# andimarafioti/qwen3-tts-cuda-graphs

Measured on NVIDIA B200. Metric: audio_seconds_per_second, higher is better.
Workload: dtype bf16

## Files before the change

### qwen3_tts_cuda_graphs_b200/csrc/fq3_kernel.cuh

```cuda
#pragma once
#include "fq3_common.cuh"

namespace fq3 {

__device__ __forceinline__ uint32_t smem_u32(const void* p) { return (uint32_t)__cvta_generic_to_shared(p); }

__device__ __forceinline__ void mbar_init(uint64_t* bar, uint32_t count) {
  asm volatile("mbarrier.init.shared::cta.b64 [%0], %1;" ::"r"(smem_u32(bar)), "r"(count) : "memory");
}
__device__ __forceinline__ void mbar_arrive(uint64_t* bar) {
  asm volatile("mbarrier.arrive.shared::cta.b64 _, [%0];" ::"r"(smem_u32(bar)) : "memory");
}
__device__ __forceinline__ void mbar_arrive_expect_tx(uint64_t* bar, uint32_t bytes) {
  asm volatile("mbarrier.arrive.expect_tx.shared::cta.b64 _, [%0], %1;" ::"r"(smem_u32(bar)), "r"(bytes) : "memory");
}
__device__ __forceinline__ bool mbar_try_wait(uint64_t* bar, uint32_t parity) {
  uint32_t ok;
  asm volatile(
      "{\n\t.reg .pred p;\n\t"
      "mbarrier.try_wait.parity.shared::cta.b64 p, [%1], %2;\n\t"
      "selp.u32 %0, 1, 0, p;\n\t}"
      : "=r"(ok)
      : "r"(smem_u32(bar)), "r"(parity)
      : "memory");
// ... 37 lines not shown
  return t;
}
__device__ __forceinline__ int ld_volatile_shared_i32(const int* p) {
  int v;
  asm volatile("ld.volatile.shared.s32 %0, [%1];" : "=r"(v) : "r"(smem_u32(p)) : "memory");
  return v;
}
__device__ __forceinline__ void st_volatile_shared_i32(int* p, int v) {
  asm volatile("st.volatile.shared.s32 [%0], %1;" ::"r"(smem_u32(p)), "r"(v) : "memory");
}
__device__ __forceinline__ uint4 lds128(uint32_t addr) {
  uint4 v;
  asm volatile("ld.shared.v4.u32 {%0, %1, %2, %3}, [%4];" : "=r"(v.x), "=r"(v.y), "=r"(v.z), "=r"(v.w) : "r"(addr));
  return v;
}

__device__ __forceinline__ LLWord ll_ld(const LLWord* p) {
  LLWord w;
  asm volatile("ld.relaxed.gpu.global.v2.u32 {%0, %1}, [%2];" : "=r"(w.x), "=r"(w.y) : "l"(p) : "memory");
  return w;
}
__device__ __forceinline__ void ll_ld2(const LLWord* p, LLWord& a, LLWord& b) {
  asm volatile("ld.relaxed.gpu.global.v4.u32 {%0, %1, %2, %3}, [%4];" : "=r"(a.x), "=r"(a.y), "=r"(b.x), "=r"(b.y) : "l"(p) : "memory");
}
__device__ __forceinline__ void ll_st(LLWord* p, uint32_t payload, uint32_t ep) {
  const unsigned long long val = ((unsigned long long)ep << 32) | payload;
  asm volatile("red.relaxed.gpu.global.max.u64 [%0], %1;" ::"l"(p), "l"(val) : "memory");
}
__device__ __forceinline__ void ll_st2(LLWord* p, uint32_t pay0, uint32_t pay1, uint32_t ep) {
  ll_st(p, pay0, ep);
  ll_st(p + 1, pay1, ep);
}
__device__ __forceinline__ void ll_stf(LLWord* p, float v, uint32_t ep) { ll_st(p, __float_as_uint(v), ep); }

__device__ __forceinline__ float bf16r(float x) { return __bfloat162float(__float2bfloat16_rn(x)); }
__device__ __forceinline__ float bf_lo(uint32_t w) { return __uint_as_float(w << 16); }
__device__ __forceinline__ float bf_hi(uint32_t w) { return __uint_as_float(w & 0xffff0000u); }
__device__ __forceinline__ uint32_t pack_bf16x2(float lo, float hi) {
  __nv_bfloat162 v = __floats2bfloat162_rn(lo, hi);
  return *reinterpret_cast<uint32_t*>(&v);
}
__device__ __forceinline__ float warp_sum(float v) {
#pragma unroll
  for (int o = 16; o > 0; o >>= 1) v += __shfl_xor_sync(0xffffffffu, v, o);
  return v;
}
__device__ __forceinline__ float warp_max(float v) {
#pragma unroll
  for (int o = 16; o > 0; o >>= 1) v = fmaxf(v, __shfl_xor_sync(0xffffffffu, v, o));
  return v;
}
struct Smem {
  uint64_t* full;
  uint64_t* empty;
  int* ctl;
  float* red;
  unsigned char* scratch;
  KindDesc* kinds;
  UnitDesc* units;
  Phase* prog;
  unsigned char* gam;
  unsigned char* xbuf;
  unsigned char* ring;
};

__device__ __forceinline__ Smem carve_smem(unsigned char* base, const LaunchParams& p) {
// ... 407 lines not shown
  cbar_sync();
  if (tprof) prof_acc(p, 2, *tprof);
}

template <int UNITS, int JC>
__device__ __noinline__ void load_x_rows(const LaunchParams& p, uint32_t flags, const LLWord* in, int ld, uint32_t gam, float eps,
                                         int K, int M, uint32_t ep_in, int pidx, uint32_t xs, uint32_t red) {
  load_x_rows_impl<UNITS, JC, false>(p, flags, in, ld, gam, eps, K, M, ep_in, pidx, xs, red, nullptr);
}

__device__ __forceinline__ float2 tree_parts(float y0, float y1, uint32_t pa, uint32_t stride, int wpg) {
  float P0[8], P1[8];
#pragma unroll
  for (int g = 0; g < 8; ++g) {
    float s0 = 0.f, s1 = 0.f;
    if (g != 0 && g < wpg) { const float2 v = lds_f32x2(pa + (uint32_t)g * stride); s0 = v.x; s1 = v.y; }
    if (g + 8 < wpg) { const float2 v = lds_f32x2(pa + (uint32_t)(g + 8) * stride); s0 += v.x; s1 += v.y; }
    if (g == 0) { s0 += y0; s1 += y1; }
    P0[g] = s0; P1[g] = s1;
  }
  return make_float2(((P0[0] + P0[1]) + (P0[2] + P0[3])) + ((P0[4] + P0[5]) + (P0[6] + P0[7])),
                     ((P1[0] + P1[1]) + (P1[2] + P1[3])) + ((P1[4] + P1[5]) + (P1[6] + P1[7])));
}

template <bool PROF>
__device__ __forceinline__ void gemv_phase_consume(const Ctx& c, const Phase& ph, const LaunchParams& p, RingCur& cur, RingCur& gcur, uint32_t& gst,
                                                   int pidx, uint32_t ep) {
  const int tid = threadIdx.x, warp = tid >> 5, lane = tid & 31;
  RingCur cur0 = cur, gcur0 = gcur;
  const uint32_t kda = c.kinds + (uint32_t)ph.kind * (uint32_t)sizeof(KindDesc);
  const uint4 k0 = lds128(kda);
  const uint4 k3 = lds128(kda + 48u);
  const uint4 ud = lds128(c.units + (uint32_t)(ph.kind * kConsumerWarps + warp) * (uint32_t)sizeof(UnitDesc));
  if (k3.x == 0u) return;
  const uint32_t flags = k0.w;
  const int Kq = (int)k0.z;
  const LLWord* in = reinterpret_cast<const LLWord*>(((unsigned long long)k0.y << 32) | k0.x);
  const uint32_t ep_in = (pidx == 0 && ep == p.epoch_base + 1) ? 0u : ep - 1;
  const bool norm = (flags & F_PRENORM) != 0;
  if (PROF) prof_mark(p, pidx, 0);
  if (PROF) prof_cta_time(p, pidx, 0);
  if (PROF) prof_warp_time(p, pidx, 0);

  const uint4 k6 = lds128(kda + 96u);
  const bool fast = k6.w != 0u;
  const bool poller = tid < kPollThreads;
  const bool have0 = poller && tid < Kq, have1 = poller && tid + kPollThreads < Kq, have2 = poller && tid + 2 * kPollThreads < Kq;
  const LLWord* src = in + 2 * tid;
  uint4 w0 = make_uint4(0u, ep_in, 0u, ep_in), w1 = w0, w2 = w0;
  if (fast) {
    if (have0) w0 = ll_ld_pair(src);
    if (have1) w1 = ll_ld_pair(src + 2 * kPollThreads);
    if (have2) w2 = ll_ld_pair(src + 4 * kPollThreads);
  }

  const uint4 k1 = lds128(kda + 16u);
  const uint4 k2 = lds128(kda + 32u);
  const uint4 k4 = lds128(kda + 64u);
  const uint4 k5 = lds128(kda + 80u);
  const int M = (int)k6.x, n_words = (int)k6.y, K = (int)k6.z;
  FQ3_ASSERT(M >= 1 && M <= kMaxRows && (K & 63) == 0 && (M == 1 ? 2 * K * 2 : M * (int)xrow_stride(K)) <= p.xbuf_bytes, pidx, 300000 + M);
  struct { int g, grp0, n_stages; } sb = {(int)k3.x, (int)k3.y, (int)k4.w};
  const int wpg = (int)k3.z, gpr = (int)k3.w, spg = (int)k4.x, ro_shift = (int)k4.z;
  const int g8 = lane >> 2, t = lane & 3;
  const int wgrp = (int)ud.x, kp = (int)ud.y;
  const bool w_act = wgrp < gpr;
  int ch0 = (int)ud.z, ch1 = (int)ud.w;
  uint32_t gsrc = c.gam + (uint32_t)gcur0.slot * (uint32_t)c.gam_bytes + (uint32_t)tid * 8u;
  uint32_t gfullb = c.gfull + (uint32_t)gcur0.slot * 8u, gemptyb = c.gempty + (uint32_t)gcur0.slot * 8u;
  const uint32_t glap = gcur0.lap;
  if (norm) gcur0.advance(1, kGammaSlots);
  float eps = __uint_as_float(k5.x);
  float inv_k = __uint_as_float(k5.y);
  const uint32_t par = gst & 1u;
  const uint32_t xs = c.xs + (fast ? par * c.xhalf : 0u);
  uint32_t xdst0 = xs + xquad_off(tid), xdst1 = xs + xquad_off(tid + kPollThreads), xdst2 = xs + xquad_off(tid + 2 * kPollThreads);
  uint32_t xrow = xs + (uint32_t)min(g8, M - 1) * xrow_stride(K) + (uint32_t)t * 16u;
  const uint32_t lane_w = (uint32_t)lane * 16u;
  const uint32_t pbase = c.scratch + par * (uint32_t)(kConsumerWarps * 32 * 8);
  uint32_t pdst = pbase + (uint32_t)((wgrp * wpg + kp) * 32 + lane) * 8u;
  LLWord* out = reinterpret_cast<LLWord*>(((unsigned long long)k1.y << 32) | k1.x);
  const LLWord* resp = reinterpret_cast<const LLWord*>(((unsigned long long)k1.w << 32) | k1.z);
  const uint32_t* biasp = reinterpret_cast<const uint32_t*>(((unsigned long long)k2.y << 32) | k2.x);
  const int ldout = (int)k2.z, ldres = (int)k2.w;
  const bool f_lane = w_act && kp == 0 && g8 < M && (ro_shift == 1 || (t & 1) == 0);
  const int f_sub = (ro_shift == 1) ? t : (t >> 1);
  const int wpgrp = (int)k5.w;
  int gi = wgrp;
  int f_word = (sb.grp0 + gi) * wpgrp + f_sub;
  uint32_t res0 = 0u, bias0 = 0u;
  const bool g_ok0 = w_act && gi < sb.g;
  if (f_lane && g_ok0 && f_word < n_words) {
    if (flags & F_RESID) res0 = ll_ld(resp + (size_t)g8 * ldres + f_word).x;
    if (flags & F_BIAS) bias0 = __ldg(biasp + f_word);
// ... 77 lines not shown
          const float4 r0 = lds_f32x4(c.red), r1 = lds_f32x4(c.red + 16u);
          static_assert(kPollWarps == 8, "the RMSNorm reduction reads eight per-warp sums");
          tot = ((r0.x + r0.y) + (r0.z + r0.w)) + ((r1.x + r1.y) + (r1.z + r1.w));
        }
        const float rs = rsqrtf(fmaf(tot, inv_k, eps));
        const bool wr = (flags & F_WRITE_NORMED) && blockIdx.x == 0;
        if (have0) {
          const uint32_t y0 = norm_pair(w0.x, rs, g0.x), y1 = norm_pair(w0.z, rs, g0.y);
          xquad_store(xdst0, y0, y1);
          if (wr) reinterpret_cast<uint2*>(p.bufs[BUF_HID])[tid] = make_uint2(y0, y1);
        }
        if (have1) {
          const uint32_t y0 = norm_pair(w1.x, rs, g1.x), y1 = norm_pair(w1.z, rs, g1.y);
          xquad_store(xdst1, y0, y1);
          if (wr) reinterpret_cast<uint2*>(p.bufs[BUF_HID])[tid + kPollThreads] = make_uint2(y0, y1);
        }
        if (have2) {
          const uint32_t y0 = norm_pair(w2.x, rs, g2.x), y1 = norm_pair(w2.z, rs, g2.y);
          xquad_store(xdst2, y0, y1);
          if (wr) reinterpret_cast<uint2*>(p.bufs[BUF_HID])[tid + 2 * kPollThreads] = make_uint2(y0, y1);
        }
        __syncwarp();
        if (lane == 0) mbar_arrive_a(gemptyb);
      }
    }
    if (PROF) prof_warp_time(p, pidx, 6);
    cbar_sync();
    if (PROF) prof_warp_time(p, pidx, 1);
  } else {
    if (norm && !mbar_try_wait_a(gfullb, glap)) {
      Spin spin;
      while (!mbar_try_wait_a(gfullb, glap)) spin.tick(p, DE_FULL_WAIT, pidx, 100);
    }
    load_x_rows<1, 3>(p, flags, in, (int)lds_u32(kda + 112u), gsrc - (uint32_t)tid * 8u, eps, K, M, ep_in, pidx, c.xs, c.red);
    if (norm) {
      if (lane == 0) mbar_arrive_a(gemptyb);
    }
  }
  if (PROF) prof_mark(p, pidx, 1);

#pragma unroll 1
  for (int r = 0; r < n_rounds; ++r) {
    if (r != 0) cbar_sync();
    gi = r * gpr + wgrp;
    if (!(w_act && gi < sb.g)) continue;
    if (r != 0) {
      my = cur0;
      my.advance(gi * spg + (ch0 >> 5), c.n_stages);
      const uint32_t fb = c.full + (uint32_t)my.slot * 8u;
      Spin spin;
      while (!mbar_try_wait_a(fb, my.lap)) spin.tick(p, DE_FULL_WAIT, pidx, my.slot);
      wa0 = c.ring + lane_w + (uint32_t)my.slot * kStageBytes + (uint32_t)(ch0 & (kStageChunks - 1)) * kBlockBytes;
    }
    float acc[4] = {0.f, 0.f, 0.f, 0.f}, acc2[4] = {0.f, 0.f, 0.f, 0.f};
    int ch = ch0;
    uint32_t wa = wa0, xa = xa0;
    if (PROF && r == 0) prof_mark(p, pidx, 8);
    if (PROF && r == 0) prof_warp_time(p, pidx, 2);
    if (r == 0 && npre > 0) {
      uint4 xv = lds128(xa);
#pragma unroll
      for (int i = 0; i < kPre; ++i) {
        if (i < npre) {
          uint4 xn = xv;
          if (ch0 + i + 1 < ch1) xn = lds128(xa + (uint32_t)(i + 1) * kXBlock);
          mma_bf16(acc, xv.x, xv.x, xv.y, xv.y, wreg[i].x, wreg[i].y);
          mma_bf16(acc2, xv.z, xv.z, xv.w, xv.w, wreg[i].z, wreg[i].w);
// ... 81 lines not shown
#pragma unroll
            for (int o = 4; o <= 16; o <<= 1) {
              s0 += __shfl_xor_sync(0xffffffffu, s0, o);
              s1 += __shfl_xor_sync(0xffffffffu, s1, o);
            }
            if (g8 == m) { r0 = s0; r1 = s1; }
          }
          y0 = r0; y1 = r1;
        }
      }
    }
    if (PROF && r == 0) prof_mark(p, pidx, 10, kProfLeader);
    if (kp == 0) {
      if (r != 0) {
        f_word = (sb.grp0 + gi) * wpgrp + f_sub;
        if (f_lane && f_word < n_words) {
          if (flags & F_RESID) res0 = ll_ld(resp + (size_t)g8 * ldres + f_word).x;
          if (flags & F_BIAS) bias0 = __ldg(biasp + f_word);
        }
      }
      float lo, hi;
      if (flags & F_SWIGLU) {
        const float e = bf16r(bf16r(silu_f(bf16r(y0))) * bf16r(y1));
        lo = e;
        hi = __shfl_down_sync(0xffffffffu, e, 1);
      } else {
        lo = y0; hi = y1;
        if (flags & F_BIAS) { lo += bf_lo(bias0); hi += bf_hi(bias0); }
        lo = bf16r(lo); hi = bf16r(hi);
        if (flags & F_SILU) { lo = bf16r(silu_f(lo)); hi = bf16r(silu_f(hi)); }
      }
      if (flags & F_RESID) { lo = bf16r(bf_lo(res0) + lo); hi = bf16r(bf_hi(res0) + hi); }
      if (PROF) prof_cta_time(p, pidx, 1);
      if (f_lane && f_word < n_words) ll_st(out + (size_t)g8 * ldout + f_word, pack_bf16x2(lo, hi), ep);
      if (PROF && r == 0) prof_mark(p, pidx, 11, kProfLeader);
      if (PROF && r == 0) prof_warp_time(p, pidx, 7);
      if (wpg == 1) {
        __syncwarp();
        if (lane == 0) {
          int rs = cur0.slot + gi * spg;
          while (rs >= c.n_stages) rs -= c.n_stages;
          for (int s2 = 0; s2 < spg; ++s2) {
            mbar_arrive_a(c.empty + (uint32_t)rs * 8u);
            if (++rs == c.n_stages) rs = 0;
          }
        }
      }
    }
  }
  cur0.advance(sb.n_stages, c.n_stages);
  cur = cur0;
  gcur = gcur0;
  gst = ((gst & 1u) ^ 1u) | (fast ? 0u : 2u);
  if (PROF) prof_mark(p, pidx, 3, kProfLeader);
  if (PROF) prof_warp_time(p, pidx, 4);
}


struct KindRegs {
  const LLWord* in; int Kq, flags; LLWord* out; const LLWord* res; const uint32_t* bias; int ldout, ldres;
  int g, grp0, wpg, gpr, spg, nch, ro_shift, n_stages; float eps, inv_k; int n_rounds, wpgrp, M, n_words, K, fast, ldin, norm;
};
__device__ __forceinline__ KindRegs load_kind(uint32_t kda) {
  const uint4 k0 = lds128(kda), k1 = lds128(kda + 16u), k2 = lds128(kda + 32u), k3 = lds128(kda + 48u), k4 = lds128(kda + 64u),
              k5 = lds128(kda + 80u), k6 = lds128(kda + 96u), k7 = lds128(kda + 112u);
  KindRegs r;
  r.in = reinterpret_cast<const LLWord*>(((unsigned long long)k0.y << 32) | k0.x); r.Kq = (int)k0.z; r.flags = (int)k0.w;
// ... 274 lines not shown
__device__ __forceinline__ int num_splits(int L, int cap) {
  const int want = (L + kSplitLen - 1) / kSplitLen;
  return max(1, min(want, cap));
}

struct RopeRegs {
  uint2 g2, c2, s2;
};
__device__ __forceinline__ RopeRegs rope_load(const bf16* gamma, const bf16* cosp, const bf16* sinp, int lane) {
  RopeRegs r;
  const uint64_t keep = policy_evict_last();
  r.g2 = ldg_keep_u2(gamma + lane * 4, keep);
  r.c2 = ldg_keep_u2(cosp + lane * 4, keep);
  r.s2 = ldg_keep_u2(sinp + lane * 4, keep);
  return r;
}
__device__ __forceinline__ void head_norm_rope(float (&x)[4], const RopeRegs& rr, float eps, int lane) {
  const uint2 g2 = rr.g2, c2 = rr.c2, s2 = rr.s2;
  float ss = x[0] * x[0] + x[1] * x[1] + x[2] * x[2] + x[3] * x[3];
  ss = warp_sum(ss);
  const float rs = rsqrtf(ss * (1.f / kHeadDim) + eps);
  const float g[4] = {bf_lo(g2.x), bf_hi(g2.x), bf_lo(g2.y), bf_hi(g2.y)};
  const float c[4] = {bf_lo(c2.x), bf_hi(c2.x), bf_lo(c2.y), bf_hi(c2.y)};
  const float sn[4] = {bf_lo(s2.x), bf_hi(s2.x), bf_lo(s2.y), bf_hi(s2.y)};
  float y[4];
#pragma unroll
  for (int i = 0; i < 4; ++i) y[i] = bf16r(bf16r(x[i] * rs) * g[i]);
#pragma unroll
  for (int i = 0; i < 4; ++i) {
    const float partner = __shfl_xor_sync(0xffffffffu, y[i], 16);
    const float rot = (lane < 16) ? -partner : partner;
    x[i] = bf16r(bf16r(y[i] * c[i]) + bf16r(rot * sn[i]));
  }
}

__device__ __forceinline__ void ll_head_wait(const LLWord* src, uint32_t ep, LLWord& a, LLWord& b, const LaunchParams& p, int phase) {
  ll_ld2(src, a, b);
  if (ep == 0) return;
  Spin spin;
  unsigned tries = 0;
  while (__any_sync(0xffffffffu, a.y != ep || b.y != ep)) {
    if (++tries > 4) __nanosleep(40);
    spin.tick(p, DE_LL_WAIT, phase, (int)ep);
    ll_ld2(src, a, b);
  }
}

constexpr int kGq = 2;
constexpr int kAttnPre = 2;
constexpr int kAttnShort = 2 * kAttnPre * kConsumerWarps;

template <bool PROF>
__device__ __forceinline__ void attn_row(const Phase& ph, const LaunchParams& p, unsigned char* smem_base, const Group& gr, int r, int kvh, int sp,
                                      int nsplit, uint32_t ep, int pidx) {
  const Smem sm = carve_smem(smem_base, p);
  const StackRt& S = p.stacks[ph.stack];
  const int warp = threadIdx.x >> 5, lane = threadIdx.x & 31;
  const int gq = S.nq / S.nkv;
  const int qb = ph.stack == ST_TALKER ? BUF_TQKV : BUF_PQKV, ab = ph.stack == ST_TALKER ? BUF_TATT : BUF_PATT;
  const LLWord* qkv = reinterpret_cast<const LLWord*>(p.bufs[qb]) + (size_t)gr.first_row * p.ld[qb];
  const int ldq = p.ld[qb];
  constexpr int HW = kHeadDim / 2;
  const size_t head_base = (((size_t)ph.layer * S.n_slots + gr.slot) * S.nkv + kvh) * (size_t)S.max_pos * kHeadDim;
  bf16* Kc = S.kcache + head_base;
  bf16* Vc = S.vcache + head_base;
  const int pos = gr.pos0 + r;
// ... 2 lines not shown
  FQ3_ASSERT(r >= 0 && r < kMaxRows && sp >= 0 && sp < nsplit && nsplit <= kMaxSplits, pidx, 210000 + sp);
  const int per = (L + nsplit - 1) / nsplit;
  const int a = gr.n_pad + sp * per;
  const int b = min(a + per, pos + 1);
  float* qs = reinterpret_cast<float*>(sm.scratch);
  uint4* fresh = reinterpret_cast<uint4*>(sm.scratch + 1024);
  float* wp = reinterpret_cast<float*>(sm.scratch + 1024 + 4096);
  const uint32_t ep_in = ep - 1;
  const int hw = lane >> 4, dl = lane & 15;
  if (PROF) prof_mark(p, pidx, 0);

  uint4 kpre[kAttnPre], vpre[kAttnPre];
#pragma unroll
  for (int u = 0; u < kAttnPre; ++u) {
    const int i = a + warp * 2 + hw + u * 2 * kConsumerWarps;
    kpre[u] = make_uint4(0u, 0u, 0u, 0u);
    vpre[u] = kpre[u];
    if (i < b && i < gr.pos0) {
      kpre[u] = __ldcg(reinterpret_cast<const uint4*>(Kc + (size_t)i * kHeadDim) + dl);
      vpre[u] = __ldcg(reinterpret_cast<const uint4*>(Vc + (size_t)i * kHeadDim) + dl);
    }
  }
  cbar_sync();
  if (threadIdx.x < kGq * kAttnShort) wp[threadIdx.x] = -INFINITY;

  for (int it = warp; it < gq + 2 * (r + 1); it += kConsumerWarps) {
    if (it < gq) {
      const int rp = min(max(pos + gr.rope_delta, 0), S.rope_len - 1);
      const LLWord* src = qkv + (size_t)r * ldq + (kvh * gq + it) * HW + lane * 2;
      const RopeRegs rr = rope_load(reinterpret_cast<const bf16*>(p.arena + (size_t)ph.g_off * 16), S.rope_cos + (size_t)rp * kHeadDim,
                                    S.rope_sin + (size_t)rp * kHeadDim, lane);
      LLWord w0, w1;
      ll_head_wait(src, ep_in, w0, w1, p, pidx);
      float x[4] = {bf_lo(w0.x), bf_hi(w0.x), bf_lo(w1.x), bf_hi(w1.x)};
      head_norm_rope(x, rr, S.eps, lane);
      const float scale = rsqrtf((float)kHeadDim);
      *reinterpret_cast<float4*>(qs + it * kHeadDim + lane * 4) = make_float4(x[0] * scale, x[1] * scale, x[2] * scale, x[3] * scale);
    } else {
      const int r2 = (it - gq) >> 1;
      const bool is_v = ((it - gq) & 1) != 0;
      const int kp = gr.pos0 + r2;
      if (kp >= a && kp < b) {
        const LLWord* row = qkv + (size_t)r2 * ldq;
        uint2* f = reinterpret_cast<uint2*>(fresh + (size_t)r2 * 32);
        if (is_v) {
          const LLWord* vsrc = row + (S.nq + S.nkv + kvh) * HW + lane * 2;
          LLWord v0, v1;
          ll_head_wait(vsrc, ep_in, v0, v1, p, pidx);
          const uint2 vv = make_uint2(v0.x, v1.x);
          *reinterpret_cast<uint2*>(Vc + (size_t)kp * kHeadDim + lane * 4) = vv;
          f[32 + lane] = vv;
        } else {
          const int rp = min(max(kp + gr.rope_delta, 0), S.rope_len - 1);
          const LLWord* ksrc = row + (S.nq + kvh) * HW + lane * 2;
          const RopeRegs rr = rope_load(reinterpret_cast<const bf16*>(p.arena + (size_t)ph.b_off * 16), S.rope_cos + (size_t)rp * kHeadDim,
                                        S.rope_sin + (size_t)rp * kHeadDim, lane);
          LLWord k0, k1;
          ll_head_wait(ksrc, ep_in, k0, k1, p, pidx);
          float x[4] = {bf_lo(k0.x), bf_hi(k0.x), bf_lo(k1.x), bf_hi(k1.x)};
          head_norm_rope(x, rr, S.eps, lane);
          const uint2 kk = make_uint2(pack_bf16x2(x[0], x[1]), pack_bf16x2(x[2], x[3]));
          *reinterpret_cast<uint2*>(Kc + (size_t)kp * kHeadDim + lane * 4) = kk;
          f[lane] = kk;
        }
      }
    }
  }
  cbar_sync();
  if (PROF) prof_mark(p, pidx, 1);

  float qr[kGq][8];
#pragma unroll
  for (int j = 0; j < kGq; ++j) {
    const float4 q0 = *reinterpret_cast<const float4*>(qs + j * kHeadDim + dl * 8);
    const float4 q1 = *reinterpret_cast<const float4*>(qs + j * kHeadDim + dl * 8 + 4);
    qr[j][0] = q0.x; qr[j][1] = q0.y; qr[j][2] = q0.z; qr[j][3] = q0.w;
    qr[j][4] = q1.x; qr[j][5] = q1.y; qr[j][6] = q1.z; qr[j][7] = q1.w;
  }
  if (b - a <= kAttnShort) {
    float* sc = wp;
    uint4* vst = reinterpret_cast<uint4*>(wp + kGq * kAttnShort);
    float sv[2][kGq];
    uint4 vv[2];
    int idx[2];
#pragma unroll
    for (int u = 0; u < 2; ++u) {
      const int i = a + warp * 2 + hw + u * 2 * kConsumerWarps;
      idx[u] = (i < b) ? i - a : -1;
      uint4 kk = make_uint4(0u, 0u, 0u, 0u);
      vv[u] = kk;
      if (i < b) {
        if (i >= gr.pos0) {
          const uint4* f = fresh + (size_t)(i - gr.pos0) * 32;
          kk = f[dl];
          vv[u] = f[16 + dl];
        } else {
          kk = kpre[u];
          vv[u] = vpre[u];
        }
      }
      const float k[8] = {bf_lo(kk.x), bf_hi(kk.x), bf_lo(kk.y), bf_hi(kk.y), bf_lo(kk.z), bf_hi(kk.z), bf_lo(kk.w), bf_hi(kk.w)};
#pragma unroll
      for (int j = 0; j < kGq; ++j) {
        float t = 0.f;
#pragma unroll
        for (int d = 0; d < 8; ++d) t = fmaf(qr[j][d], k[d], t);
        sv[u][j] = t;
      }
    }
#pragma unroll
    for (int o = 8; o > 0; o >>= 1) {
#pragma unroll
      for (int u = 0; u < 2; ++u) {
#pragma unroll
        for (int j = 0; j < kGq; ++j) sv[u][j] += __shfl_xor_sync(0xffffffffu, sv[u][j], o);
      }
    }
#pragma unroll
    for (int u = 0; u < 2; ++u) {
      vst[(warp * 2 + hw + u * 2 * kConsumerWarps) * 16 + dl] = vv[u];
      if (idx[u] >= 0 && dl < kGq) sc[dl * kAttnShort + idx[u]] = (dl == 0) ? sv[u][0] : sv[u][1];
    }
    if (PROF) prof_mark(p, pidx, 2);
    cbar_sync();
    float* pr = reinterpret_cast<float*>(vst + kAttnShort * 16);
    const int n = b - a;
    const int n4 = (n + 3) >> 2;
    if (threadIdx.x < kGq * kAttnShort) {
      const int j = threadIdx.x / kAttnShort, i = threadIdx.x - j * kAttnShort;
      const float4* s4 = reinterpret_cast<const float4*>(sc + j * kAttnShort);
      float Mx = -INFINITY;
      for (int g4 = 0; g4 < n4; ++g4) {
        const float4 v = s4[g4];
        Mx = fmaxf(Mx, fmaxf(fmaxf(v.x, v.y), fmaxf(v.z, v.w)));
      }
      pr[threadIdx.x] = expf(sc[threadIdx.x] - Mx);
      if (i == 0) pr[kGq * kAttnShort + j] = Mx;
    }
    cbar_sync();
    if (threadIdx.x < gq * HW) {
      const int j = threadIdx.x / HW, wd = threadIdx.x - j * HW;
      const int qh = kvh * gq + j;
      const int row = gr.first_row + r;
      const float4* p4 = reinterpret_cast<const float4*>(pr + j * kAttnShort);
      const float Mx = pr[kGq * kAttnShort + j];
      const uint32_t* vw = reinterpret_cast<const uint32_t*>(vst) + wd;
      float Lsum = 0.f, O0 = 0.f, O1 = 0.f;
#pragma unroll 3
      for (int g4 = 0; g4 < n4; ++g4) {
        const float4 v = p4[g4];
        const uint32_t w0 = vw[(4 * g4) * HW], w1 = vw[(4 * g4 + 1) * HW], w2 = vw[(4 * g4 + 2) * HW], w3 = vw[(4 * g4 + 3) * HW];
        Lsum += v.x; O0 = fmaf(v.x, bf_lo(w0), O0); O1 = fmaf(v.x, bf_hi(w0), O1);
        Lsum += v.y; O0 = fmaf(v.y, bf_lo(w1), O0); O1 = fmaf(v.y, bf_hi(w1), O1);
        Lsum += v.z; O0 = fmaf(v.z, bf_lo(w2), O0); O1 = fmaf(v.z, bf_hi(w2), O1);
        Lsum += v.w; O0 = fmaf(v.w, bf_lo(w3), O0); O1 = fmaf(v.w, bf_hi(w3), O1);
      }
      if (nsplit == 1) {
        const float y0 = bf16r(Lsum > 0.f ? O0 / Lsum : 0.f), y1 = bf16r(Lsum > 0.f ? O1 / Lsum : 0.f);
        ll_st(reinterpret_cast<LLWord*>(p.bufs[ab]) + (size_t)row * p.ld[ab] + qh * HW + wd, pack_bf16x2(y0, y1), ep);
      } else {
        LLWord* dst = p.attn_part + (((size_t)row * S.nq + qh) * kMaxSplits + sp) * kPartStride;
        if (wd == 0) ll_st2(dst, __float_as_uint(Mx), __float_as_uint(Lsum), ep);
        ll_st2(dst + 4 + 2 * wd, __float_as_uint(O0), __float_as_uint(O1), ep);
      }
    }
    if (PROF) prof_mark(p, pidx, 3);
    return;
  }
  float m_run[kGq], l_run[kGq], acc[kGq][8];
#pragma unroll
  for (int j = 0; j < kGq; ++j) {
    m_run[j] = -INFINITY; l_run[j] = 0.f;
#pragma unroll
    for (int d = 0; d < 8; ++d) acc[j][d] = 0.f;
  }
  auto step = [&](const uint4& kk, const uint4& vv, bool valid) {
    const float k[8] = {bf_lo(kk.x), bf_hi(kk.x), bf_lo(kk.y), bf_hi(kk.y), bf_lo(kk.z), bf_hi(kk.z), bf_lo(kk.w), bf_hi(kk.w)};
    const float v[8] = {bf_lo(vv.x), bf_hi(vv.x), bf_lo(vv.y), bf_hi(vv.y), bf_lo(vv.z), bf_hi(vv.z), bf_lo(vv.w), bf_hi(vv.w)};
    float s[kGq];
#pragma unroll
    for (int j = 0; j < kGq; ++j) {
      float t = 0.f;
#pragma unroll
      for (int d = 0; d < 8; ++d) t = fmaf(qr[j][d], k[d], t);
      s[j] = t;
    }
#pragma unroll
    for (int o = 8; o > 0; o >>= 1) {
#pragma unroll
      for (int j = 0; j < kGq; ++j) s[j] += __shfl_xor_sync(0xffffffffu, s[j], o);
    }
    if (valid) {
#pragma unroll
      for (int j = 0; j < kGq; ++j) {
        const float m_new = fmaxf(m_run[j], s[j]);
        const float corr = expf(m_run[j] - m_new);
        const float pj = expf(s[j] - m_new);
        l_run[j] = l_run[j] * corr + pj;
#pragma unroll
        for (int d = 0; d < 8; ++d) acc[j][d] = fmaf(pj, v[d], acc[j][d] * corr);
        m_run[j] = m_new;
      }
    }
  };
  {
    int u = 0;
#pragma unroll 1
    for (int i0 = a + warp * 2; i0 < b; i0 += 2 * kConsumerWarps, ++u) {
      const int i = i0 + hw;
      const bool valid = i < b;
      uint4 kk = make_uint4(0u, 0u, 0u, 0u), vv = kk;
      if (valid) {
        if (i >= gr.pos0) {
          const uint4* f = fresh + (size_t)(i - gr.pos0) * 32;
          kk = f[dl];
          vv = f[16 + dl];
        } else if (u < kAttnPre) {
          kk = (u == 0) ? kpre[0] : kpre[1];
          vv = (u == 0) ? vpre[0] : vpre[1];
        } else {
          kk = __ldcg(reinterpret_cast<const uint4*>(Kc + (size_t)i * kHeadDim) + dl);
          vv = __ldcg(reinterpret_cast<const uint4*>(Vc + (size_t)i * kHeadDim) + dl);
        }
      }
// ... 9 lines not shown
    const float c_o = (m_o == -INFINITY) ? 0.f : expf(m_o - m_new);
    float o8[8];
#pragma unroll
    for (int d = 0; d < 8; ++d) {
      const float a_o = __shfl_xor_sync(0xffffffffu, acc[j][d], 16);
      o8[d] = acc[j][d] * c_s + a_o * c_o;
    }
    const float l_new = l_run[j] * c_s + l_o * c_o;
    if (hw == 0) {
      float* w = wp + ((size_t)warp * kGq + j) * kPartStride;
      if (dl == 0) { w[0] = m_new; w[1] = l_new; }
      *reinterpret_cast<float4*>(w + 4 + dl * 8) = make_float4(o8[0], o8[1], o8[2], o8[3]);
      *reinterpret_cast<float4*>(w + 8 + dl * 8) = make_float4(o8[4], o8[5], o8[6], o8[7]);
    }
  }
  if (PROF) prof_mark(p, pidx, 2);
  cbar_sync();
  if (threadIdx.x < gq * HW) {
    const int j = threadIdx.x / HW, wd = threadIdx.x - j * HW;
    const int qh = kvh * gq + j;
    const int row = gr.first_row + r;
    const int nw = min(kConsumerWarps, (b - a + 1) >> 1);
    float Mx = -INFINITY;
    for (int w = 0; w < nw; ++w) Mx = fmaxf(Mx, wp[((size_t)w * kGq + j) * kPartStride]);
    float Lsum = 0.f, O0 = 0.f, O1 = 0.f;
    for (int w = 0; w < nw; ++w) {
      const float* q = wp + ((size_t)w * kGq + j) * kPartStride;
      const float f = (q[0] == -INFINITY) ? 0.f : expf(q[0] - Mx);
      Lsum += q[1] * f;
      const float2 o2 = *reinterpret_cast<const float2*>(q + 4 + 2 * wd);
      O0 += o2.x * f; O1 += o2.y * f;
    }
    if (nsplit == 1) {
      const float y0 = bf16r(Lsum > 0.f ? O0 / Lsum : 0.f), y1 = bf16r(Lsum > 0.f ? O1 / Lsum : 0.f);
      ll_st(reinterpret_cast<LLWord*>(p.bufs[ab]) + (size_t)row * p.ld[ab] + qh * HW + wd, pack_bf16x2(y0, y1), ep);
    } else {
      LLWord* dst = p.attn_part + (((size_t)row * S.nq + qh) * kMaxSplits + sp) * kPartStride;
      if (wd == 0) ll_st2(dst, __float_as_uint(Mx), __float_as_uint(Lsum), ep);
      ll_st2(dst + 4 + 2 * wd, __float_as_uint(O0), __float_as_uint(O1), ep);
    }
  }
  if (PROF) prof_mark(p, pidx, 3);
}

__device__ __forceinline__ void combine_step(float& Mx, float& Lsum, float& O0, float& O1, float ms, float ls, float a0, float a1) {
  if (ms != -INFINITY) {
    const float m_new = fmaxf(Mx, ms);
    const float c_old = (Mx == -INFINITY) ? 0.f : expf(Mx - m_new);
    const float c_new = expf(ms - m_new);
    Lsum = Lsum * c_old + ls * c_new;
    O0 = O0 * c_old + a0 * c_new;
    O1 = O1 * c_old + a1 * c_new;
    Mx = m_new;
  }
}

__device__ __forceinline__ void attn_combine(const Phase& ph, const LaunchParams& p, const Group& gr, int r, int kvh, int nsplit, uint32_t ep,
                                          int pidx) {
  const StackRt& S = p.stacks[ph.stack];
  const int gq = S.nq / S.nkv;
  const int ab = ph.stack == ST_TALKER ? BUF_TATT : BUF_PATT;
  constexpr int HW = kHeadDim / 2;
  if (threadIdx.x < gq * HW) {
    const int j = threadIdx.x / HW, wd = threadIdx.x - j * HW;
    const int qh = kvh * gq + j;
    const int row = gr.first_row + r;
    const LLWord* src = p.attn_part + (((size_t)row * S.nq + qh) * kMaxSplits) * kPartStride;
    float Mx = -INFINITY, Lsum = 0.f, O0 = 0.f, O1 = 0.f;
// ... 267 lines not shown
  }
#pragma unroll 1
  for (int pass = 0; pass < 2; ++pass) {
#pragma unroll 1
    for (int item = first; item < total; item += step) {
      int base = 0;
      bool found = false;
      for (int g = 0; g < ng && !found; ++g) {
        const Group gr = get_group(ph, p, g, frame_pos);
        for (int r = 0; r < gr.nrows; ++r) {
          int nsplit; bool multi;
          const int nitems = row_items(gr, r, nsplit, multi);
          if (item < base + nitems) {
            const int it = item - base;
            if (multi) {
              if constexpr (WIDE) {
                if (pass == 0) attn_item_multi(ph, p, smem_base, gr, it, nsplit, ep, pidx);
              }
            } else {
              const int kvh = small_div(it, nsplit), sp = it - kvh * nsplit;
              if (pass == 0) attn_row<PROF>(ph, p, smem_base, gr, r, kvh, sp, nsplit, ep, pidx);
              else if (nsplit > 1 && sp == 0) attn_combine(ph, p, gr, r, kvh, nsplit, ep, pidx);
            }
            found = true;
            break;
          }
          base += nitems;
        }
      }
    }
  }
}

__device__ __forceinline__ uint32_t f2key(float f) {
  uint32_t u = __float_as_uint(f);
  return (u & 0x80000000u) ? ~u : (u | 0x80000000u);
}
__device__ __forceinline__ float key2f(uint32_t k) {
  uint32_t u = (k & 0x80000000u) ? (k & 0x7fffffffu) : ~k;
  return __uint_as_float(u);
}
__device__ __forceinline__ uint4 philox4x32_10(uint4 c, uint2 k) {
#pragma unroll
  for (int i = 0; i < 10; ++i) {
    const uint32_t hi0 = __umulhi(0xD2511F53u, c.x), lo0 = 0xD2511F53u * c.x;
    const uint32_t hi1 = __umulhi(0xCD9E8D57u, c.z), lo1 = 0xCD9E8D57u * c.z;
    c = make_uint4(hi1 ^ c.y ^ k.x, lo1, hi0 ^ c.w ^ k.y, lo0);
    k.x += 0x9E3779B9u;
    k.y += 0xBB67AE85u;
  }
  return c;
}

struct SampleScratch {
  float* sl;
  unsigned* hist;
  float* redf;
  int* redi;
};
__device__ __forceinline__ SampleScratch sample_scratch(unsigned char* scratch) {
  SampleScratch s;
  s.sl = reinterpret_cast<float*>(scratch);
  s.hist = reinterpret_cast<unsigned*>(scratch + 20 * 1024);
  s.redf = reinterpret_cast<float*>(scratch + 21 * 1024);
  s.redi = reinterpret_cast<int*>(scratch + 21 * 1024 + 256);
  return s;
// ... 729 lines not shown
          int* sconst = reinterpret_cast<int*>(smem_raw + kStreamConstOffset);
          sconst[tid] = __ldcg(&st->n_pad);
          sconst[kMaxWide + tid] = __ldcg(&st->rope_delta);
        } else {
          done = (int)ll_wait(&st->ctl[0], ep0, p, -2);
          pos = (int)ll_wait(&st->ctl[1], ep0, p, -2);
        }
        frame_pos[tid] = pos;
        frame_done[tid] = done;
      }
      cbar_sync();
      if (p.mode == MODE_FRAMES && iter > 0) {
        int all_done = 1;
        for (int b = 0; b < p.n_rows; ++b) all_done &= (frame_done[b] != 0);
        if (all_done) {
          if (tid == 0) st_volatile_shared_i32(&sm.ctl[0], -1);
          break;
        }
      }
    }
    for (int i = 0; i < p.n_phases; ++i) {
      const Phase ph = load_phase(sm.prog, i);
      const uint32_t ep = ep0 + (uint32_t)i + 1u;
      switch (ph.type) {
        case PH_GEMV:
          if constexpr (WIDE) gemv_phase_consume_wide(c, ph, p, cur, gcur, gst, i, ep);
          else gemv_phase_consume<PROF>(c, ph, p, cur, gcur, gst, i, ep);
          break;
        case PH_ATTN:
          if constexpr (WIDE) {
            long long tp = (FQ3_WIDE_PROF && p.prof) ? clock64() : 0ll;
            attn_phase<PROF, true>(ph, p, smem_raw, ep, i, frame_pos);
            prof_acc(p, 4, tp);
          } else {
            attn_phase<PROF, false>(ph, p, smem_raw, ep, i, frame_pos);
          }
          break;
        case PH_SAMPLE:
          if constexpr (WIDE) {
            long long tp = (FQ3_WIDE_PROF && p.prof) ? clock64() : 0ll;
            sample_phase<WIDE>(ph, p, smem_raw, ep, i, frame_done);
            prof_acc(p, 5, tp);
          } else {
            sample_phase<WIDE>(ph, p, smem_raw, ep, i, frame_done);
          }
          break;
        default: if (tid == 0) device_fault(p, DE_BAD_PHASE, i, ph.type); break;
      }
    }
  }
}

__global__ void fq3_tile_weights_kernel(const bf16* __restrict__ W, uint4* __restrict__ out, int N, int K) {
  const long pieces = (long)((N + 7) / 8) * K;
  for (long idx = blockIdx.x * (long)blockDim.x + threadIdx.x; idx < pieces; idx += (long)gridDim.x * blockDim.x) {
    const long grp = idx / K;
    const int pc = (int)(idx - grp * K);
    const int ch = pc >> 5, ln = pc & 31, r8 = ln >> 2, t = ln & 3;
    const long row = grp * 8 + r8;
    uint4 v = make_uint4(0u, 0u, 0u, 0u);
    if (row < N) {
      const uint32_t* src = reinterpret_cast<const uint32_t*>(W + (size_t)row * K + ch * kChunkK) + t;
      v = make_uint4(__ldg(src), __ldg(src + 4), __ldg(src + 8), __ldg(src + 12));
    }
    out[idx] = v;
  }
// ... 182 lines not shown
```

Before: 46.31.

## Fold predictor attention into the following GEMV by staging outputs in shared memory

Adds a pred_attn_fold path for the predictor stack in single-row decode mode. Every CTA redundantly computes the short-context attention for all KV heads and writes the result directly into the shared-memory x buffer of the next GEMV phase. Flag bits in gst make that GEMV skip its global polling and x loading, and add an acq_rel fence before stores so the KV-cache writes are ordered. This removes a global LL write/poll round trip and a phase boundary, at the cost of redundant attention compute in every CTA. It also factors existing attention helpers into shared inline functions.

```diff
diff --git a/qwen3_tts_cuda_graphs_b200/csrc/fq3_kernel.cuh b/qwen3_tts_cuda_graphs_b200/csrc/fq3_kernel.cuh
--- a/qwen3_tts_cuda_graphs_b200/csrc/fq3_kernel.cuh
+++ b/qwen3_tts_cuda_graphs_b200/csrc/fq3_kernel.cuh
@@ -93,6 +93,9 @@
   ll_st(p + 1, pay1, ep);
 }
 __device__ __forceinline__ void ll_stf(LLWord* p, float v, uint32_t ep) { ll_st(p, __float_as_uint(v), ep); }
+
+__device__ __forceinline__ void fence_acq_rel_gpu() { asm volatile("fence.acq_rel.gpu;" ::: "memory"); }
+__device__ __forceinline__ void prefetch_l1(const void* ptr) { asm volatile("prefetch.global.L1 [%0];" ::"l"(ptr)); }
 
 __device__ __forceinline__ float bf16r(float x) { return __bfloat162float(__float2bfloat16_rn(x)); }
 __device__ __forceinline__ float bf_lo(uint32_t w) { return __uint_as_float(w << 16); }
@@ -566,7 +569,10 @@
   const uint4 k0 = lds128(kda);
   const uint4 k3 = lds128(kda + 48u);
   const uint4 ud = lds128(c.units + (uint32_t)(ph.kind * kConsumerWarps + warp) * (uint32_t)sizeof(UnitDesc));
-  if (k3.x == 0u) return;
+  if (k3.x == 0u) {
+    gst &= 3u;
+    return;
+  }
   const uint32_t flags = k0.w;
   const int Kq = (int)k0.z;
   const LLWord* in = reinterpret_cast<const LLWord*>(((unsigned long long)k0.y << 32) | k0.x);
@@ -578,7 +584,8 @@
 
   const uint4 k6 = lds128(kda + 96u);
   const bool fast = k6.w != 0u;
-  const bool poller = tid < kPollThreads;
+  const bool staged = (gst & 4u) != 0u;
+  const bool poller = !staged && tid < kPollThreads;
   const bool have0 = poller && tid < Kq, have1 = poller && tid + kPollThreads < Kq, have2 = poller && tid + 2 * kPollThreads < Kq;
   const LLWord* src = in + 2 * tid;
   uint4 w0 = make_uint4(0u, ep_in, 0u, ep_in), w1 = w0, w2 = w0;
@@ -593,7 +600,7 @@
   const uint4 k4 = lds128(kda + 64u);
   const uint4 k5 = lds128(kda + 80u);
   const int M = (int)k6.x, n_words = (int)k6.y, K = (int)k6.z;
-  FQ3_ASSERT(M >= 1 && M <= kMaxRows && (K & 63) == 0 && (M == 1 ? 2 * K * 2 : M * (int)xrow_stride(K)) <= p.xbuf_bytes, pidx, 300000 + M);
+  FQ3_ASSERT(M >= 1 && M <= kMaxRows && (K & 63) == 0 && (M == 1 ? 2 * K * 2 : M * (int)xrow_stride(K)) <= p.xbuf_bytes && !(staged && norm), pidx, 300000 + M);
   struct { int g, grp0, n_stages; } sb = {(int)k3.x, (int)k3.y, (int)k4.w};
   const int wpg = (int)k3.z, gpr = (int)k3.w, spg = (int)k4.x, ro_shift = (int)k4.z;
   const int g8 = lane >> 2, t = lane & 3;
@@ -737,7 +744,7 @@
       Spin spin;
       while (!mbar_try_wait_a(gfullb, glap)) spin.tick(p, DE_FULL_WAIT, pidx, 100);
     }
-    load_x_rows<1, 3>(p, flags, in, (int)lds_u32(kda + 112u), gsrc - (uint32_t)tid * 8u, eps, K, M, ep_in, pidx, c.xs, c.red);
+    if (!staged) load_x_rows<1, 3>(p, flags, in, (int)lds_u32(kda + 112u), gsrc - (uint32_t)tid * 8u, eps, K, M, ep_in, pidx, c.xs, c.red);
     if (norm) {
       if (lane == 0) mbar_arrive_a(gemptyb);
     }
@@ -885,7 +892,10 @@
       }
       if (flags & F_RESID) { lo = bf16r(bf_lo(res0) + lo); hi = bf16r(bf_hi(res0) + hi); }
       if (PROF) prof_cta_time(p, pidx, 1);
-      if (f_lane && f_word < n_words) ll_st(out + (size_t)g8 * ldout + f_word, pack_bf16x2(lo, hi), ep);
+      if (f_lane && f_word < n_words) {
+        if (gst & 8u) fence_acq_rel_gpu();
+        ll_st(out + (size_t)g8 * ldout + f_word, pack_bf16x2(lo, hi), ep);
+      }
       if (PROF && r == 0) prof_mark(p, pidx, 11, kProfLeader);
       if (PROF && r == 0) prof_warp_time(p, pidx, 7);
       if (wpg == 1) {
@@ -1226,6 +1236,52 @@
     const float rot = (lane < 16) ? -partner : partner;
     x[i] = bf16r(bf16r(y[i] * c[i]) + bf16r(rot * sn[i]));
   }
+}
+
+__device__ __forceinline__ float4 q_head(LLWord w0, LLWord w1, const RopeRegs& rr, float eps, int lane) {
+  float x[4] = {bf_lo(w0.x), bf_hi(w0.x), bf_lo(w1.x), bf_hi(w1.x)};
+  head_norm_rope(x, rr, eps, lane);
+  const float scale = rsqrtf((float)kHeadDim);
+  return make_float4(x[0] * scale, x[1] * scale, x[2] * scale, x[3] * scale);
+}
+__device__ __forceinline__ uint2 k_head(LLWord k0, LLWord k1, const RopeRegs& rr, float eps, int lane) {
+  float x[4] = {bf_lo(k0.x), bf_hi(k0.x), bf_lo(k1.x), bf_hi(k1.x)};
+  head_norm_rope(x, rr, eps, lane);
+  return make_uint2(pack_bf16x2(x[0], x[1]), pack_bf16x2(x[2], x[3]));
+}
+__device__ __forceinline__ float qk_partial(const float (&q)[8], uint4 kk) {
+  const float k[8] = {bf_lo(kk.x), bf_hi(kk.x), bf_lo(kk.y), bf_hi(kk.y), bf_lo(kk.z), bf_hi(kk.z), bf_lo(kk.w), bf_hi(kk.w)};
+  float t = 0.f;
+#pragma unroll
+  for (int d = 0; d < 8; ++d) t = fmaf(q[d], k[d], t);
+  return t;
+}
+template <int N>
+__device__ __forceinline__ void half_sums(float (&v)[N]) {
+#pragma unroll
+  for (int o = 8; o > 0; o >>= 1) {
+#pragma unroll
+    for (int n = 0; n < N; ++n) v[n] += __shfl_xor_sync(0xffffffffu, v[n], o);
+  }
+}
+__device__ __forceinline__ float scores_max(const float* sc, int n4) {
+  const float4* s4 = reinterpret_cast<const float4*>(sc);
+  float Mx = -INFINITY;
+  for (int g4 = 0; g4 < n4; ++g4) {
+    const float4 v = s4[g4];
+    Mx = fmaxf(Mx, fmaxf(fmaxf(v.x, v.y), fmaxf(v.z, v.w)));
+  }
+  return Mx;
+}
+__device__ __forceinline__ void pv_step4(float4 v, uint32_t w0, uint32_t w1, uint32_t w2, uint32_t w3, float& Lsum, float& O0, float& O1) {
+  Lsum += v.x; O0 = fmaf(v.x, bf_lo(w0), O0); O1 = fmaf(v.x, bf_hi(w0), O1);
+  Lsum += v.y; O0 = fmaf(v.y, bf_lo(w1), O0); O1 = fmaf(v.y, bf_hi(w1), O1);
+  Lsum += v.z; O0 = fmaf(v.z, bf_lo(w2), O0); O1 = fmaf(v.z, bf_hi(w2), O1);
+  Lsum += v.w; O0 = fmaf(v.w, bf_lo(w3), O0); O1 = fmaf(v.w, bf_hi(w3), O1);
+}
+__device__ __forceinline__ uint32_t attn_word(float Lsum, float O0, float O1) {
+  const float y0 = bf16r(Lsum > 0.f ? O0 / Lsum : 0.f), y1 = bf16r(Lsum > 0.f ? O1 / Lsum : 0.f);
+  return pack_bf16x2(y0, y1);
 }
 
 __device__ __forceinline__ void ll_head_wait(const LLWord* src, uint32_t ep, LLWord& a, LLWord& b, const LaunchParams& p, int phase) {
@@ -1294,10 +1350,7 @@
                                     S.rope_sin + (size_t)rp * kHeadDim, lane);
       LLWord w0, w1;
       ll_head_wait(src, ep_in, w0, w1, p, pidx);
-      float x[4] = {bf_lo(w0.x), bf_hi(w0.x), bf_lo(w1.x), bf_hi(w1.x)};
-      head_norm_rope(x, rr, S.eps, lane);
-      const float scale = rsqrtf((float)kHeadDim);
-      *reinterpret_cast<float4*>(qs + it * kHeadDim + lane * 4) = make_float4(x[0] * scale, x[1] * scale, x[2] * scale, x[3] * scale);
+      *reinterpret_cast<float4*>(qs + it * kHeadDim + lane * 4) = q_head(w0, w1, rr, S.eps, lane);
     } else {
       const int r2 = (it - gq) >> 1;
       const bool is_v = ((it - gq) & 1) != 0;
@@ -1319,9 +1372,7 @@
                                         S.rope_sin + (size_t)rp * kHeadDim, lane);
           LLWord k0, k1;
           ll_head_wait(ksrc, ep_in, k0, k1, p, pidx);
-          float x[4] = {bf_lo(k0.x), bf_hi(k0.x), bf_lo(k1.x), bf_hi(k1.x)};
-          head_norm_rope(x, rr, S.eps, lane);
-          const uint2 kk = make_uint2(pack_bf16x2(x[0], x[1]), pack_bf16x2(x[2], x[3]));
+          const uint2 kk = k_head(k0, k1, rr, S.eps, lane);
           *reinterpret_cast<uint2*>(Kc + (size_t)kp * kHeadDim + lane * 4) = kk;
           f[lane] = kk;
         }
@@ -1342,7 +1393,7 @@
   if (b - a <= kAttnShort) {
     float* sc = wp;
     uint4* vst = reinterpret_cast<uint4*>(wp + kGq * kAttnShort);
-    float sv[2][kGq];
+    float sv[2 * kGq];
     uint4 vv[2];
     int idx[2];
 #pragma unroll
@@ -1361,27 +1412,14 @@
           vv[u] = vpre[u];
         }
       }
-      const float k[8] = {bf_lo(kk.x), bf_hi(kk.x), bf_lo(kk.y), bf_hi(kk.y), bf_lo(kk.z), bf_hi(kk.z), bf_lo(kk.w), bf_hi(kk.w)};
-#pragma unroll
-      for (int j = 0; j < kGq; ++j) {
-        float t = 0.f;
-#pragma unroll
-        for (int d = 0; d < 8; ++d) t = fmaf(qr[j][d], k[d], t);
-        sv[u][j] = t;
-      }
-    }
-#pragma unroll
-    for (int o = 8; o > 0; o >>= 1) {
-#pragma unroll
-      for (int u = 0; u < 2; ++u) {
-#pragma unroll
-        for (int j = 0; j < kGq; ++j) sv[u][j] += __shfl_xor_sync(0xffffffffu, sv[u][j], o);
-      }
-    }
+#pragma unroll
+      for (int j = 0; j < kGq; ++j) sv[u * kGq + j] = qk_partial(qr[j], kk);
+    }
+    half_sums(sv);
 #pragma unroll
     for (int u = 0; u < 2; ++u) {
       vst[(warp * 2 + hw + u * 2 * kConsumerWarps) * 16 + dl] = vv[u];
-      if (idx[u] >= 0 && dl < kGq) sc[dl * kAttnShort + idx[u]] = (dl == 0) ? sv[u][0] : sv[u][1];
+      if (idx[u] >= 0 && dl < kGq) sc[dl * kAttnShort + idx[u]] = (dl == 0) ? sv[u * kGq] : sv[u * kGq + 1];
     }
     if (PROF) prof_mark(p, pidx, 2);
     cbar_sync();
@@ -1390,12 +1428,7 @@
     const int n4 = (n + 3) >> 2;
     if (threadIdx.x < kGq * kAttnShort) {
       const int j = threadIdx.x / kAttnShort, i = threadIdx.x - j * kAttnShort;
-      const float4* s4 = reinterpret_cast<const float4*>(sc + j * kAttnShort);
-      float Mx = -INFINITY;
-      for (int g4 = 0; g4 < n4; ++g4) {
-        const float4 v = s4[g4];
-        Mx = fmaxf(Mx, fmaxf(fmaxf(v.x, v.y), fmaxf(v.z, v.w)));
-      }
+      const float Mx = scores_max(sc + j * kAttnShort, n4);
       pr[threadIdx.x] = expf(sc[threadIdx.x] - Mx);
       if (i == 0) pr[kGq * kAttnShort + j] = Mx;
     }
@@ -1409,17 +1442,10 @@
       const uint32_t* vw = reinterpret_cast<const uint32_t*>(vst) + wd;
       float Lsum = 0.f, O0 = 0.f, O1 = 0.f;
 #pragma unroll 3
-      for (int g4 = 0; g4 < n4; ++g4) {
-        const float4 v = p4[g4];
-        const uint32_t w0 = vw[(4 * g4) * HW], w1 = vw[(4 * g4 + 1) * HW], w2 = vw[(4 * g4 + 2) * HW], w3 = vw[(4 * g4 + 3) * HW];
-        Lsum += v.x; O0 = fmaf(v.x, bf_lo(w0), O0); O1 = fmaf(v.x, bf_hi(w0), O1);
-        Lsum += v.y; O0 = fmaf(v.y, bf_lo(w1), O0); O1 = fmaf(v.y, bf_hi(w1), O1);
-        Lsum += v.z; O0 = fmaf(v.z, bf_lo(w2), O0); O1 = fmaf(v.z, bf_hi(w2), O1);
-        Lsum += v.w; O0 = fmaf(v.w, bf_lo(w3), O0); O1 = fmaf(v.w, bf_hi(w3), O1);
-      }
+      for (int g4 = 0; g4 < n4; ++g4)
+        pv_step4(p4[g4], vw[(4 * g4) * HW], vw[(4 * g4 + 1) * HW], vw[(4 * g4 + 2) * HW], vw[(4 * g4 + 3) * HW], Lsum, O0, O1);
       if (nsplit == 1) {
-        const float y0 = bf16r(Lsum > 0.f ? O0 / Lsum : 0.f), y1 = bf16r(Lsum > 0.f ? O1 / Lsum : 0.f);
-        ll_st(reinterpret_cast<LLWord*>(p.bufs[ab]) + (size_t)row * p.ld[ab] + qh * HW + wd, pack_bf16x2(y0, y1), ep);
+        ll_st(reinterpret_cast<LLWord*>(p.bufs[ab]) + (size_t)row * p.ld[ab] + qh * HW + wd, attn_word(Lsum, O0, O1), ep);
       } else {
         LLWord* dst = p.attn_part + (((size_t)row * S.nq + qh) * kMaxSplits + sp) * kPartStride;
         if (wd == 0) ll_st2(dst, __float_as_uint(Mx), __float_as_uint(Lsum), ep);
@@ -1437,21 +1463,11 @@
     for (int d = 0; d < 8; ++d) acc[j][d] = 0.f;
   }
   auto step = [&](const uint4& kk, const uint4& vv, bool valid) {
-    const float k[8] = {bf_lo(kk.x), bf_hi(kk.x), bf_lo(kk.y), bf_hi(kk.y), bf_lo(kk.z), bf_hi(kk.z), bf_lo(kk.w), bf_hi(kk.w)};
     const float v[8] = {bf_lo(vv.x), bf_hi(vv.x), bf_lo(vv.y), bf_hi(vv.y), bf_lo(vv.z), bf_hi(vv.z), bf_lo(vv.w), bf_hi(vv.w)};
     float s[kGq];
 #pragma unroll
-    for (int j = 0; j < kGq; ++j) {
-      float t = 0.f;
-#pragma unroll
-      for (int d = 0; d < 8; ++d) t = fmaf(qr[j][d], k[d], t);
-      s[j] = t;
-    }
-#pragma unroll
-    for (int o = 8; o > 0; o >>= 1) {
-#pragma unroll
-      for (int j = 0; j < kGq; ++j) s[j] += __shfl_xor_sync(0xffffffffu, s[j], o);
-    }
+    for (int j = 0; j < kGq; ++j) s[j] = qk_partial(qr[j], kk);
+    half_sums(s);
     if (valid) {
 #pragma unroll
       for (int j = 0; j < kGq; ++j) {
@@ -1527,8 +1543,7 @@
       O0 += o2.x * f; O1 += o2.y * f;
     }
     if (nsplit == 1) {
-      const float y0 = bf16r(Lsum > 0.f ? O0 / Lsum : 0.f), y1 = bf16r(Lsum > 0.f ? O1 / Lsum : 0.f);
-      ll_st(reinterpret_cast<LLWord*>(p.bufs[ab]) + (size_t)row * p.ld[ab] + qh * HW + wd, pack_bf16x2(y0, y1), ep);
+      ll_st(reinterpret_cast<LLWord*>(p.bufs[ab]) + (size_t)row * p.ld[ab] + qh * HW + wd, attn_word(Lsum, O0, O1), ep);
     } else {
       LLWord* dst = p.attn_part + (((size_t)row * S.nq + qh) * kMaxSplits + sp) * kPartStride;
       if (wd == 0) ll_st2(dst, __float_as_uint(Mx), __float_as_uint(Lsum), ep);
@@ -1862,6 +1877,152 @@
   }
 }
 
+constexpr int kFoldWarpBytes = 2048;
+constexpr int kFoldPos = 32;
+static_assert(kConsumerWarps * kFoldWarpBytes <= kScratchBytes && 1024 + 2 * kGq * kFoldPos * 4 <= kFoldWarpBytes, "fold scratch");
+template <bool PROF>
+__device__ __forceinline__ void pred_attn_fold(const Ctx& c, const Phase& ph, const LaunchParams& p, unsigned char* smem_base, uint32_t& gst,
+                                               uint32_t ep, int pidx) {
+  const StackRt& S = p.stacks[ST_PRED];
+  uint32_t tid_v, cta_v;
+  asm volatile("mov.u32 %0, %%tid.x;" : "=r"(tid_v));
+  asm volatile("mov.u32 %0, %%ctaid.x;" : "=r"(cta_v));
+  const int warp = (int)tid_v >> 5, lane = (int)tid_v & 31, hw = lane >> 4, dl = lane & 15, cta = (int)cta_v;
+  const Group gr = get_group(ph, p, 0, nullptr);
+  const int n_items = gr.nrows * S.nkv;
+  const LLWord* qkv = reinterpret_cast<const LLWord*>(p.bufs[BUF_PQKV]);
+  const int ldq = p.ld[BUF_PQKV];
+  constexpr int HW = kHeadDim / 2;
+  const uint32_t ep_in = ep - 1;
+  const Phase nx = load_phase(c.prog, pidx + 1);
+  const uint32_t kda = c.kinds + (uint32_t)nx.kind * (uint32_t)sizeof(KindDesc);
+  const uint4 k6 = lds128(kda + 96u);
+  const uint32_t xs = c.xs + (k6.w ? (gst & 1u) * c.xhalf : 0u), rstride = xrow_stride((int)k6.z);
+  FQ3_ASSERT(nx.type == PH_GEMV && nx.in_buf == BUF_PATT && !(nx.flags & F_PRENORM) && (int)k6.x == gr.nrows && (int)k6.z == S.nq * kHeadDim &&
+                 S.nq == kGq * S.nkv && gr.pos0 + gr.nrows <= kFoldPos && gr.nrows <= 2 && (cta >= S.nkv || lds_u32(kda + 48u) != 0u),
+             pidx, 230000 + gr.pos0);
+  if (PROF) prof_mark(p, pidx, 0);
+  const bool cached = gr.pos0 > 0;
+  if (cached && warp < n_items) fence_acq_rel_gpu();
+  cbar_sync();
+  unsigned char* ws = smem_base + kHeaderBytes + warp * kFoldWarpBytes;
+  uint2* kf = reinterpret_cast<uint2*>(ws);
+  uint2* vf = reinterpret_cast<uint2*>(ws + 512);
+  float* sc = reinterpret_cast<float*>(ws + 1024);
+  float* pr = sc + kGq * kFoldPos;
+#pragma unroll 1
+  for (int item = warp; item < n_items; item += kConsumerWarps) {
+    const int r = item >= S.nkv ? 1 : 0, kvh = item - r * S.nkv;
+    const int pos = gr.pos0 + r, n = pos + 1, n4 = (n + 3) >> 2;
+    const size_t head_base = (((size_t)ph.layer * S.n_slots + gr.slot) * S.nkv + kvh) * (size_t)S.max_pos * kHeadDim;
+    bf16* Kc = S.kcache + head_base;
+    bf16* Vc = S.vcache + head_base;
+    for (int l = lane; l < gr.pos0 * 4; l += 32) prefetch_l1(((l & 2) ? Vc : Kc) + (size_t)(l >> 2) * kHeadDim + (l & 1) * 64);
+    const int rpq = min(max(pos + gr.rope_delta, 0), S.rope_len - 1);
+    const RopeRegs rq = rope_load(reinterpret_cast<const bf16*>(p.arena + (size_t)ph.g_off * 16), S.rope_cos + (size_t)rpq * kHeadDim,
+                                  S.rope_sin + (size_t)rpq * kHeadDim, lane);
+    LLWord a[4], b[4];
+#pragma unroll 1
+    for (int rr = 0; rr <= r; ++rr) {
+#pragma unroll
+      for (int t = 0; t < 4; ++t) {
+        if (t >= 2 || rr == 0) {
+          const int head = t < 2 ? kvh * kGq + t : S.nq + (t == 3 ? S.nkv : 0) + kvh;
+          ll_ld2(qkv + (size_t)(t < 2 ? r : rr) * ldq + head * HW + lane * 2, a[t], b[t]);
+        }
+      }
+      Spin spin;
+      unsigned tries = 0;
+      while (true) {
+        bool bad = false;
+#pragma unroll
+        for (int t = 0; t < 4; ++t) bad |= (a[t].y != ep_in) | (b[t].y != ep_in);
+        if (!__any_sync(0xffffffffu, bad)) break;
+        if (++tries > 4) __nanosleep(40);
+        spin.tick(p, DE_LL_WAIT, pidx, (int)ep_in);
+#pragma unroll
+        for (int t = 0; t < 4; ++t) {
+          if ((a[t].y != ep_in) | (b[t].y != ep_in)) {
+            const int head = t < 2 ? kvh * kGq + t : S.nq + (t == 3 ? S.nkv : 0) + kvh;
+            ll_ld2(qkv + (size_t)(t < 2 ? r : rr) * ldq + head * HW + lane * 2, a[t], b[t]);
+          }
+        }
+      }
+      const int kp = gr.pos0 + rr, rpk = min(max(kp + gr.rope_delta, 0), S.rope_len - 1);
+      const RopeRegs rk = rope_load(reinterpret_cast<const bf16*>(p.arena + (size_t)ph.b_off * 16), S.rope_cos + (size_t)rpk * kHeadDim,
+                                    S.rope_sin + (size_t)rpk * kHeadDim, lane);
+      const uint2 kk = k_head(a[2], b[2], rk, S.eps, lane);
+      const uint2 vv = make_uint2(a[3].x, b[3].x);
+      kf[rr * 32 + lane] = kk;
+      vf[rr * 32 + lane] = vv;
+      if (rr == r && cta == kvh) {
+        *reinterpret_cast<uint2*>(Kc + (size_t)kp * kHeadDim + lane * 4) = kk;
+        *reinterpret_cast<uint2*>(Vc + (size_t)kp * kHeadDim + lane * 4) = vv;
+      }
+    }
+    if (PROF && item == 0) prof_mark(p, pidx, 1);
+    float qr[kGq][8];
+#pragma unroll
+    for (int j = 0; j < kGq; ++j) {
+      const float4 x = q_head(a[j], b[j], rq, S.eps, lane);
+#pragma unroll
+      for (int h = 0; h < 2; ++h) {
+        qr[j][4 * h + 0] = __shfl_sync(0xffffffffu, x.x, 2 * dl + h);
+        qr[j][4 * h + 1] = __shfl_sync(0xffffffffu, x.y, 2 * dl + h);
+        qr[j][4 * h + 2] = __shfl_sync(0xffffffffu, x.z, 2 * dl + h);
+        qr[j][4 * h + 3] = __shfl_sync(0xffffffffu, x.w, 2 * dl + h);
+      }
+    }
+    __syncwarp();
+#pragma unroll 2
+    for (int i0 = 0; i0 < n; i0 += 2) {
+      const int i = i0 + hw;
+      uint4 kk = make_uint4(0u, 0u, 0u, 0u);
+      if (i < n) kk = i >= gr.pos0 ? reinterpret_cast<const uint4*>(kf)[(i - gr.pos0) * 16 + dl]
+                                   : __ldca(reinterpret_cast<const uint4*>(Kc + (size_t)i * kHeadDim) + dl);
+      float sv[kGq] = {qk_partial(qr[0], kk), qk_partial(qr[1], kk)};
+      half_sums(sv);
+      if (i < n && dl < kGq) sc[dl * kFoldPos + i] = dl == 0 ? sv[0] : sv[1];
+    }
+    if (lane < kGq * 4 && n + (lane & 3) < 4 * n4) sc[(lane >> 2) * kFoldPos + n + (lane & 3)] = -INFINITY;
+    __syncwarp();
+#pragma unroll
+    for (int j = 0; j < kGq; ++j) {
+      if (lane < 4 * n4) {
+        const float Mx = scores_max(sc + j * kFoldPos, n4);
+        pr[j * kFoldPos + lane] = expf(sc[j * kFoldPos + lane] - Mx);
+      }
+    }
+    __syncwarp();
+    auto vword = [&](int i, int wd) -> uint32_t {
+      if (i >= n) return 0u;
+      if (i >= gr.pos0) return reinterpret_cast<const uint32_t*>(vf)[(i - gr.pos0) * HW + wd];
+      return __ldca(reinterpret_cast<const unsigned int*>(Vc + (size_t)i * kHeadDim) + wd);
+    };
+#pragma unroll 1
+    for (int h = 0; h < 2; ++h) {
+      const int wd = lane + 32 * h;
+      float L[kGq], O0[kGq], O1[kGq];
+#pragma unroll
+      for (int j = 0; j < kGq; ++j) { L[j] = 0.f; O0[j] = 0.f; O1[j] = 0.f; }
+#pragma unroll 1
+      for (int g4 = 0; g4 < n4; ++g4) {
+        const uint32_t w0 = vword(4 * g4, wd), w1 = vword(4 * g4 + 1, wd), w2 = vword(4 * g4 + 2, wd), w3 = vword(4 * g4 + 3, wd);
+#pragma unroll
+        for (int j = 0; j < kGq; ++j) pv_step4(reinterpret_cast<const float4*>(pr + j * kFoldPos)[g4], w0, w1, w2, w3, L[j], O0[j], O1[j]);
+      }
+#pragma unroll
+      for (int j = 0; j < kGq; ++j) {
+        const int wq = (kvh * kGq + j) * HW + wd;
+        sts_u32(xs + (uint32_t)r * rstride + xquad_off(wq >> 1) + (uint32_t)(wq & 1) * 16u, attn_word(L[j], O0[j], O1[j]));
+      }
+    }
+    __syncwarp();
+  }
+  if (PROF) prof_mark(p, pidx, 3);
+  gst |= 4u | (cta < S.nkv ? 8u : 0u);
+}
+
 __device__ __forceinline__ uint32_t f2key(float f) {
   uint32_t u = __float_as_uint(f);
   return (u & 0x80000000u) ? ~u : (u | 0x80000000u);
@@ -2657,6 +2818,8 @@
             long long tp = (FQ3_WIDE_PROF && p.prof) ? clock64() : 0ll;
             attn_phase<PROF, true>(ph, p, smem_raw, ep, i, frame_pos);
             prof_acc(p, 4, tp);
+          } else if (ph.stack == ST_PRED && p.n_rows == 1 && p.mode != MODE_PREFILL) {
+            pred_attn_fold<PROF>(c, ph, p, smem_raw, gst, ep, i);
           } else {
             attn_phase<PROF, false>(ph, p, smem_raw, ep, i, frame_pos);
           }
```

Result: slower. 35.09 (median of 6 runs) (-24.2%).
